# AmmieQi/HGNN-2

Hardware: AMD Instinct MI355X
Metric: graphs/sec forward+backward, QM9-shape batch=512, LG-GNN 5-layer d=64 (higher is better)
Workload: dtype fp32; 1 GPU; GNN_lg order 2, 5 layers, d=64, fwd+bwd, 512 QM9-shape graphs per GPU; graphs_per_gpu=512, global_batch=512, parallelism=dp1

## Files before the change

hgnn-2_amd/csrc/agg.hip:

```cpp
#include "kernels.h"

#include <initializer_list>

namespace hgnn {

template <int CPL, bool V>
__device__ __forceinline__ void load_row(const float* __restrict__ p, int C, int lane, float (&x)[CPL]) {
    const int c0 = lane * CPL;
    if constexpr (V) {
        if constexpr (CPL == 1) {
            x[0] = p[c0];
        } else if constexpr (CPL == 2) {
            const float2 v = *reinterpret_cast<const float2*>(p + c0);
            x[0] = v.x;
            x[1] = v.y;
        } else {
#pragma unroll
            for (int i = 0; i < CPL; i += 4) {
                const float4 v = *reinterpret_cast<const float4*>(p + c0 + i);
                x[i] = v.x;
                x[i + 1] = v.y;
                x[i + 2] = v.z;
                x[i + 3] = v.w;
            }
// ... 206 lines not shown
    if (a.pad_from >= 0) {
        const int kk = a.pad_from > 0 ? a.pad_from : (JT - J0) * a.cg + (CP > 0 ? 2 * a.cp : 0);
        if (lane < a.ldo - kk) o[kk + lane] = 0.f;
    }
}

template <int JT, int CG, int CP, bool V, int RPW, int J0>
__global__ void __launch_bounds__(AGG_NT) k_agg_fwd_rpw(AggFwdArgs a) {
    WaveStamp stamp(a.stamps);
    const int r0 = __builtin_amdgcn_readfirstlane((blockIdx.x * AGG_WV + (threadIdx.x >> 6)) * RPW);
    const int lane = threadIdx.x & 63;
    const int total = *a.total_rows;
    if (r0 >= total) return;
    constexpr int CGx = CG > 0 ? CG : 1, CPx = CP > 0 ? CP : 1, MX = JT > 3 ? JT - 3 : 1;
    RowInfo rgk[RPW], rpk[RPW];
#pragma unroll
    for (int k = 0; k < RPW; ++k) {
        const int r = min(r0 + k, total - 1);
        rgk[k] = RowInfo{0, 0};
        rpk[k] = RowInfo{0, 0};
        if constexpr (CG > 0) rgk[k] = row_info(a.g.rows, r);
        if constexpr (CP > 0) rpk[k] = row_info(a.p.rows, r);
    }
    LaneBn<CGx> bng;
    LaneBn<CPx> bnp;
    if constexpr (CG > 0) bng.init(a.gbn, a.cg, lane);
    if constexpr (CP > 0) bnp.init(a.pbn, a.cp, lane);
    const int stride = a.g.stride;
    float4 mgk[RPW], mpk[RPW];
    float mxk[RPW][MX];
#pragma unroll
    for (int k = 0; k < RPW; ++k) {
        mgk[k] = mpk[k] = make_float4(0.f, 0.f, 0.f, 0.f);
        const int ng = min(64, rgk[k].count), np = min(64, rpk[k].count);
        if constexpr (CG > 0) {
            mgk[k] = lane_entry(a.g.entries, stride, rgk[k].start, ng, lane);
            if constexpr (JT > 3) {
#pragma unroll
                for (int j = 3; j < JT; ++j)
                    mxk[k][j - 3] = lane < ng ? a.g.entries[(long long)(rgk[k].start + lane) * stride + 1 + j] : 0.f;
            }
        }
        if constexpr (CP > 0) mpk[k] = lane_entry(a.p.entries, 4, rpk[k].start, np, lane);
    }
#pragma unroll
    for (int k = 0; k < RPW; ++k) {
    const int r = r0 + k;
    if (r >= total) break;
    const RowInfo rg = rgk[k], rp = rpk[k];
    float* o = a.out + (long long)r * a.ldo;
    float acc[JT][CGx], am[CPx], ad[CPx];
#pragma unroll
    for (int j = 0; j < JT; ++j)
#pragma unroll
        for (int i = 0; i < CGx; ++i) acc[j][i] = 0.f;
#pragma unroll
    for (int i = 0; i < CPx; ++i) am[i] = ad[i] = 0.f;
    const int nmax = max(rg.count, rp.count);
    bool dfound = false;
    for (int e0 = 0; e0 < nmax; e0 += 64) {
        const int ng = min(64, max(0, rg.count - e0)), np = min(64, max(0, rp.count - e0));
        float4 mg = mgk[k], mp = mpk[k];
        float mx[MX];
#pragma unroll
        for (int j = 0; j < MX; ++j) mx[j] = mxk[k][j];
        if (e0 > 0) {
            if constexpr (CG > 0) {
                mg = lane_entry(a.g.entries, stride, rg.start + e0, ng, lane);
                if constexpr (JT > 3) {
#pragma unroll
                    for (int j = 3; j < JT; ++j)
                        mx[j - 3] = lane < ng ? a.g.entries[(long long)(rg.start + e0 + lane) * stride + 1 + j] : 0.f;
                }
            }
            if constexpr (CP > 0) mp = lane_entry(a.p.entries, 4, rp.start + e0, np, lane);
        }
        if constexpr (J0 > 0 && CG > 0)
            if (a.diag) diag_scan(a, r, mg, ng, lane, dfound);
        const int nn = max(ng, np);
        for (int e = 0; e < nn; e += AGG_U) {
            float xg[AGG_U][CGx], v[AGG_U][JT], xp[AGG_U][CPx], vm[AGG_U], vd[AGG_U];
            if constexpr (CG > 0) {
#pragma unroll
                for (int u = 0; u < AGG_U; ++u) {
                    const int eu = max(0, min(e + u, ng - 1));
                    const int col = __builtin_amdgcn_readlane(__float_as_int(mg.x), eu);
                    const bool live = e + u < ng;
                    v[u][0] = live ? bcast(mg.y, eu) : 0.f;
                    if constexpr (JT > 1) v[u][1] = live ? bcast(mg.z, eu) : 0.f;
                    if constexpr (JT > 2) v[u][2] = live ? bcast(mg.w, eu) : 0.f;
#pragma unroll
                    for (int j = 3; j < JT; ++j) v[u][j] = live ? bcast(mx[j - 3], eu) : 0.f;
                    if (ng > 0) load_row<CG, V>(a.xg + (long long)col * a.cg, a.cg, lane, xg[u]);
                    else
#pragma unroll
                        for (int i = 0; i < CG; ++i) xg[u][i] = 0.f;
                }
            }
            if constexpr (CP > 0) {
#pragma unroll
                for (int u = 0; u < AGG_U; ++u) {
                    const int eu = max(0, min(e + u, np - 1));
                    const int col = __builtin_amdgcn_readlane(__float_as_int(mp.x), eu);
                    const bool live = e + u < np;
                    vm[u] = live ? bcast(mp.y, eu) : 0.f;
                    vd[u] = live ? bcast(mp.z, eu) : 0.f;
                    if (np > 0) load_row<CP, V>(a.xp + (long long)col * a.cp, a.cp, lane, xp[u]);
                    else
#pragma unroll
                        for (int i = 0; i < CP; ++i) xp[u][i] = 0.f;
                }
            }
            if constexpr (CG > 0) {
#pragma unroll
                for (int u = 0; u < AGG_U; ++u) bng.apply(xg[u]);
#pragma unroll
                for (int u = 0; u < AGG_U; ++u)
#pragma unroll
                    for (int j = J0; j < JT; ++j)
#pragma unroll
                        for (int i = 0; i < CG; ++i) acc[j][i] = fmaf(v[u][j], xg[u][i], acc[j][i]);
            }
            if constexpr (CP > 0) {
#pragma unroll
                for (int u = 0; u < AGG_U; ++u) bnp.apply(xp[u]);
#pragma unroll
                for (int u = 0; u < AGG_U; ++u)
#pragma unroll
                    for (int i = 0; i < CP; ++i) {
                        am[i] = fmaf(vm[u], xp[u][i], am[i]);
                        ad[i] = fmaf(vd[u], xp[u][i], ad[i]);
                    }
            }
        }
    }
    if constexpr (CG > 0) {
#pragma unroll
        for (int j = J0; j < JT; ++j) store_row<CG, V>(o + (j - J0) * a.cg, a.cg, lane, acc[j]);
        if constexpr (J0 > 0)
            if (a.diag && !dfound && lane == 0) a.diag[r] = make_float2(0.f, 0.f);
    }
    if constexpr (CP > 0) {
        const int base = (JT - J0) * a.cg;
        store_row<CP, V>(o + base, a.cp, lane, am);
        store_row<CP, V>(o + base + a.cp, a.cp, lane, ad);
    }
    if (a.pad_from >= 0) {
        const int kk = a.pad_from > 0 ? a.pad_from : (JT - J0) * a.cg + (CP > 0 ? 2 * a.cp : 0);
        if (lane < a.ldo - kk) o[kk + lane] = 0.f;
    }
    }
}

static int cpl_of(int c) {
    if (c <= 0) return 0;
    if (c <= 64) return 1;
    if (c <= 128) return 2;
    if (c <= 256) return 4;
    if (c <= 512) return 8;
    return -1;
}

template <int JT, int CG, int CP, int J0>
static void agg_fwd_v(const AggFwdArgs& a0, dim3 g, hipStream_t s) {
    AggFwdArgs a = a0;
    const int kk = (JT - J0) * a.cg + (CP > 0 ? 2 * a.cp : 0);
    const bool v = (CG == 0 || vec_ok(CG, a.cg, a.xg, {})) && (CP == 0 || vec_ok(CP, a.cp, a.xp, {})) &&
                   (CG == 0 || vec_ok(CG, a.cg, a.out, {a.ldo, (long long)kk})) &&
                   (CP == 0 || vec_ok(CP, a.cp, a.out, {a.ldo, (long long)(JT - J0) * a.cg, (long long)a.cp}));
    const int rpw = switches().agg_rpw == 3 ? 2 : switches().agg_rpw;
    if constexpr (JT == 3) {
        if (rpw > 1) {
            const dim3 g2(ceil_div(a.cap_rows, rpw * AGG_WV));
            a.stamps = clock_stamps((long long)g2.x * AGG_WV);
            if (rpw == 4) {
                if (v) HGNN_KLAUNCH((k_agg_fwd_rpw<JT, CG, CP, true, 4, J0>), g2, dim3(AGG_NT), 0, s, a);
                else HGNN_KLAUNCH((k_agg_fwd_rpw<JT, CG, CP, false, 4, J0>), g2, dim3(AGG_NT), 0, s, a);
            } else {
                if (v) HGNN_KLAUNCH((k_agg_fwd_rpw<JT, CG, CP, true, 2, J0>), g2, dim3(AGG_NT), 0, s, a);
                else HGNN_KLAUNCH((k_agg_fwd_rpw<JT, CG, CP, false, 2, J0>), g2, dim3(AGG_NT), 0, s, a);
            }
            return;
        }
    }
    a.stamps = clock_stamps((long long)g.x * AGG_WV);
    if (v) HGNN_KLAUNCH((k_agg_fwd<JT, CG, CP, true, J0>), g, dim3(AGG_NT), 0, s, a);
    else HGNN_KLAUNCH((k_agg_fwd<JT, CG, CP, false, J0>), g, dim3(AGG_NT), 0, s, a);
}

template <int JT, int CG, int CP>
static int agg_fwd_j0(const AggFwdArgs& a, dim3 g, hipStream_t s) {
    if (a.j0 == 2) {
        if constexpr (CG > 0 && CG <= 4 && (CP == 0 || CP == CG)) {
            agg_fwd_v<JT, CG, CP, 2>(a, g, s);
            return 0;
        }
        return 2;
    }
    agg_fwd_v<JT, CG, CP, 0>(a, g, s);
    return 0;
}

template <int JT, int CG>
static int agg_fwd_cp(const AggFwdArgs& a, dim3 g, hipStream_t s) {
    int r = 0;
    switch (cpl_of(a.xp ? a.cp : 0)) {
        case 0: r = agg_fwd_j0<JT, CG, 0>(a, g, s); break;
        case 1: r = agg_fwd_j0<JT, CG, 1>(a, g, s); break;
        case 2: r = agg_fwd_j0<JT, CG, 2>(a, g, s); break;
        case 4: r = agg_fwd_j0<JT, CG, 4>(a, g, s); break;
        case 8: r = agg_fwd_j0<JT, CG, 8>(a, g, s); break;
        default: return 2;
    }
    if (r) return r;
    HGNN_LAUNCH_CHECK();
    return 0;
}

template <int JT>
static int agg_fwd_cg(const AggFwdArgs& a, dim3 g, hipStream_t s) {
    switch (cpl_of(a.xg ? a.cg : 0)) {
        case 0:
            if (!a.xp) return 2;
            return agg_fwd_cp<JT, 0>(a, g, s);
        case 1: return agg_fwd_cp<JT, 1>(a, g, s);
        case 2: return agg_fwd_cp<JT, 2>(a, g, s);
        case 4: return agg_fwd_cp<JT, 4>(a, g, s);
        case 8: return agg_fwd_cp<JT, 8>(a, g, s);
        default: return 2;
    }
}

int launch_agg_fwd(const AggFwdArgs& a, hipStream_t s) {
    if (a.cap_rows <= 0) return 0;
    if (a.j0 != 0 && (a.j0 != 2 || !a.xg || (a.diag && !a.err))) return HGNN_ERR_ARG;
    const dim3 g(ceil_div(a.cap_rows, AGG_WV));
    switch (a.jtot) {
        case 3: return agg_fwd_cg<3>(a, g, s);
        case 4: return agg_fwd_cg<4>(a, g, s);
        case 5: return agg_fwd_cg<5>(a, g, s);
        case 6: return agg_fwd_cg<6>(a, g, s);
        case 7: return agg_fwd_cg<7>(a, g, s);
        default: return 2;
    }
}

template <int JT, int C, bool V, int UB>
__device__ __forceinline__ void agg_bwd_g_chunk(const AggBwdArgs& a, float4 me, const float (&mx)[JT > 3 ? JT - 3 : 1],
                                                int n, int lane, float (&acc)[C]) {
    for (int e = 0; e < n; e += UB) {
        float x[UB][JT][C], v[UB][JT];
#pragma unroll
        for (int u = 0; u < UB; ++u) {
            const int eu = min(e + u, n - 1);
            const int col = __builtin_amdgcn_readlane(__float_as_int(me.x), eu);
            const bool live = e + u < n;
            v[u][0] = live ? bcast(me.y, eu) : 0.f;
            if constexpr (JT > 1) v[u][1] = live ? bcast(me.z, eu) : 0.f;
            if constexpr (JT > 2) v[u][2] = live ? bcast(me.w, eu) : 0.f;
#pragma unroll
            for (int j = 3; j < JT; ++j) v[u][j] = live ? bcast(mx[j - 3], eu) : 0.f;
            const float* src = a.ing + (long long)col * a.ldg + a.gofs;
#pragma unroll
            for (int j = 0; j < JT; ++j) {
                if (v[u][j] != 0.f) {
                    load_row<C, V>(src + j * a.c, a.c, lane, x[u][j]);
                } else {
#pragma unroll
                    for (int i = 0; i < C; ++i) x[u][j][i] = 0.f;
                }
            }
        }
#pragma unroll
        for (int u = 0; u < UB; ++u)
#pragma unroll
            for (int j = 0; j < JT; ++j)
#pragma unroll
                for (int i = 0; i < C; ++i) acc[i] = fmaf(v[u][j], x[u][j][i], acc[i]);
    }
}

constexpr int AGG_LONG = 8;

template <int JT, int C, bool V>
__device__ __forceinline__ void agg_bwd_g(const AggBwdArgs& a, int r, int lane) {
    float acc[C];
    float* o = a.out + (long long)r * a.ldo;
    if (a.accumulate) {
        load_row<C, V>(o, a.c, lane, acc);
    } else {
#pragma unroll
        for (int i = 0; i < C; ++i) acc[i] = 0.f;
    }
    const RowInfo ri = row_info(a.g.rows, r);
    const int stride = a.g.stride;
    for (int e0 = 0; e0 < ri.count; e0 += 64) {
        const int n = min(64, ri.count - e0);
        const float4 me = lane_entry(a.g.entries, stride, ri.start + e0, n, lane);
        float mx[JT > 3 ? JT - 3 : 1];
        mx[0] = 0.f;
        if constexpr (JT > 3) {
#pragma unroll
            for (int j = 3; j < JT; ++j)
                mx[j - 3] = lane < n ? a.g.entries[(long long)(ri.start + e0 + lane) * stride + 1 + j] : 0.f;
        }
        if (n > AGG_LONG) agg_bwd_g_chunk<JT, C, V, AGG_LONG>(a, me, mx, n, lane, acc);
        else agg_bwd_g_chunk<JT, C, V, 4>(a, me, mx, n, lane, acc);
    }
    store_row<C, V>(o, a.c, lane, acc);
}

template <int C, bool V>
__device__ __forceinline__ void agg_bwd_p(const AggBwdArgs& a, int r, int lane) {
    float acc[C];
    float* o = a.out + (long long)r * a.ldo;
    if (a.accumulate) {
        load_row<C, V>(o, a.c, lane, acc);
    } else {
#pragma unroll
        for (int i = 0; i < C; ++i) acc[i] = 0.f;
    }
    const RowInfo ri = row_info(a.p.rows, r);
    for (int e0 = 0; e0 < ri.count; e0 += 64) {
        const int n = min(64, ri.count - e0);
        const float4 me = lane_entry(a.p.entries, 4, ri.start + e0, n, lane);
        for (int e = 0; e < n; e += AGG_U) {
            float xm[AGG_U][C], xd[AGG_U][C], vm[AGG_U], vd[AGG_U];
#pragma unroll
            for (int u = 0; u < AGG_U; ++u) {
                const int eu = min(e + u, n - 1);
                const int col = __builtin_amdgcn_readlane(__float_as_int(me.x), eu);
                const bool live = e + u < n;
                vm[u] = live ? bcast(me.y, eu) : 0.f;
                vd[u] = live ? bcast(me.z, eu) : 0.f;
                const float* src = a.inp + (long long)col * a.ldp;
                load_row<C, V>(src + a.pofs_m, a.c, lane, xm[u]);
                load_row<C, V>(src + a.pofs_d, a.c, lane, xd[u]);
            }
#pragma unroll
            for (int u = 0; u < AGG_U; ++u)
#pragma unroll
                for (int i = 0; i < C; ++i) acc[i] = fmaf(vd[u], xd[u][i], fmaf(vm[u], xm[u][i], acc[i]));
        }
    }
    store_row<C, V>(o, a.c, lane, acc);
}

template <int JT, int CG, int CP, bool V, int MODE>
__global__ void __launch_bounds__(AGG_NT) k_agg_bwd(AggBwdArgs ga, AggBwdArgs pa, int gb) {
    WaveStamp stamp(ga.stamps);
    const int lane = threadIdx.x & 63;
    const int wv = threadIdx.x >> 6;
    if (MODE == 1 || (MODE == 3 && (int)blockIdx.x < gb)) {
        if constexpr (MODE != 2) {
            const int r = __builtin_amdgcn_readfirstlane((int)blockIdx.x * AGG_WV + wv);
            if (r >= *ga.total_rows) return;
            agg_bwd_g<JT, CG, V>(ga, r, lane);
        }
    } else {
        if constexpr (MODE != 1) {
            const int r = __builtin_amdgcn_readfirstlane(((int)blockIdx.x - (MODE == 3 ? gb : 0)) * AGG_WV + wv);
            if (r >= *pa.total_rows) return;
            agg_bwd_p<CP, V>(pa, r, lane);
        }
    }
}

static bool bwd_vec_g(int cpl, const AggBwdArgs& a) {
    return vec_ok(cpl, a.c, a.ing, {a.ldg, a.gofs}) && vec_ok(cpl, a.c, a.out, {a.ldo});
}
static bool bwd_vec_p(int cpl, const AggBwdArgs& a) {
    return vec_ok(cpl, a.c, a.inp, {a.ldp, a.pofs_m, a.pofs_d}) && vec_ok(cpl, a.c, a.out, {a.ldo});
}

template <int JT, int C>
static int agg_bwd_single(const AggBwdArgs& a0, hipStream_t s) {
    const dim3 g(ceil_div(a0.cap_rows, AGG_WV));
    AggBwdArgs a = a0;
    a.stamps = clock_stamps((long long)g.x * AGG_WV);
    if (a.ing) {
        if (bwd_vec_g(C, a)) HGNN_KLAUNCH((k_agg_bwd<JT, C, C, true, 1>), g, dim3(AGG_NT), 0, s, a, a, 0);
        else HGNN_KLAUNCH((k_agg_bwd<JT, C, C, false, 1>), g, dim3(AGG_NT), 0, s, a, a, 0);
    } else {
        if (bwd_vec_p(C, a)) HGNN_KLAUNCH((k_agg_bwd<3, C, C, true, 2>), g, dim3(AGG_NT), 0, s, a, a, 0);
        else HGNN_KLAUNCH((k_agg_bwd<3, C, C, false, 2>), g, dim3(AGG_NT), 0, s, a, a, 0);
    }
    HGNN_LAUNCH_CHECK();
    return 0;
}

template <int JT>
static int agg_bwd_c(const AggBwdArgs& a, hipStream_t s) {
    switch (cpl_of(a.c)) {
        case 1: return agg_bwd_single<JT, 1>(a, s);
        case 2: return agg_bwd_single<JT, 2>(a, s);
        case 4: return agg_bwd_single<JT, 4>(a, s);
        case 8: return agg_bwd_single<JT, 8>(a, s);
        default: return 2;
    }
}

int launch_agg_bwd(const AggBwdArgs& a, hipStream_t s) {
    if (a.cap_rows <= 0) return 0;
    if ((a.ing != nullptr) == (a.inp != nullptr)) return 1;
    switch (a.jtot) {
        case 3: return agg_bwd_c<3>(a, s);
        case 4: return agg_bwd_c<4>(a, s);
        case 5: return agg_bwd_c<5>(a, s);
        case 6: return agg_bwd_c<6>(a, s);
        case 7: return agg_bwd_c<7>(a, s);
        default: return 2;
    }
}

template <int JT, int C>
static int agg_bwd_pair_c(const AggBwdArgs& ga0, const AggBwdArgs& pa, hipStream_t s) {
    const int gb = ceil_div(ga0.cap_rows, AGG_WV), pb = ceil_div(pa.cap_rows, AGG_WV);
    AggBwdArgs ga = ga0;
    ga.stamps = clock_stamps((long long)(gb + pb) * AGG_WV);
    HGNN_KLAUNCH((k_agg_bwd<JT, C, C, true, 3>), dim3(gb + pb), dim3(AGG_NT), 0, s, ga, pa, gb);
    HGNN_LAUNCH_CHECK();
    return 0;
}

template <int JT>
static int agg_bwd_pair_j(const AggBwdArgs& ga, const AggBwdArgs& pa, hipStream_t s) {
    switch (cpl_of(ga.c)) {
        case 1: return agg_bwd_pair_c<JT, 1>(ga, pa, s);
        case 2: return agg_bwd_pair_c<JT, 2>(ga, pa, s);
        case 4: return agg_bwd_pair_c<JT, 4>(ga, pa, s);
        case 8: return agg_bwd_pair_c<JT, 8>(ga, pa, s);
        default: return 2;
    }
}

int launch_agg_bwd_pair(const AggBwdArgs& ga, const AggBwdArgs& pa, hipStream_t s) {
    const int cpl = cpl_of(ga.c);
    const bool pair = ga.ing && !ga.inp && pa.inp && !pa.ing && ga.cap_rows > 0 && pa.cap_rows > 0 &&
                      cpl > 0 && cpl == cpl_of(pa.c) && ga.jtot == pa.jtot && bwd_vec_g(cpl, ga) &&
                      bwd_vec_p(cpl, pa);
    if (!pair) {
        int r = launch_agg_bwd(ga, s);
        if (r) return r;
        return launch_agg_bwd(pa, s);
    }
    switch (ga.jtot) {
        case 3: return agg_bwd_pair_j<3>(ga, pa, s);
        case 4: return agg_bwd_pair_j<4>(ga, pa, s);
        case 5: return agg_bwd_pair_j<5>(ga, pa, s);
        case 6: return agg_bwd_pair_j<6>(ga, pa, s);
        case 7: return agg_bwd_pair_j<7>(ga, pa, s);
        default: return 2;
    }
}

}
```

hgnn-2_amd/csrc/bn.hip:

```cpp
#include <algorithm>

#include "kernels.h"

namespace hgnn {

__device__ __forceinline__ double block_sum_d(double v, double* red) {
    v = wave_sum_d(v);
    const int w = threadIdx.x >> 6;
    __syncthreads();
    if ((threadIdx.x & 63) == 0) red[w] = v;
    __syncthreads();
    double t = 0.0;
    const int nw = blockDim.x >> 6;
    for (int i = 0; i < nw; ++i) t += red[i];
    return t;
}

__global__ void __launch_bounds__(256) k_bn_finalize(BnFwdArgs a) {
    WaveStamp stamp(a.stamps);
    const int lane = threadIdx.x & 63;
    const int ch = blockIdx.x * 4 + (threadIdx.x >> 6);
    if (ch >= a.c) return;
    if (!a.training) {
        if (lane == 0) {
// ... 40 lines not shown
            pq[u] = in ? p[2] : 0.f;
        }
    };
    double n = 0.0, sm = 0.0;
    for (int t0 = 0; t0 < tiles; t0 += 64 * U) {
        load(t0);
#pragma unroll
        for (int u = 0; u < U; ++u) {
            n += (double)pn[u];
            sm = fma((double)pn[u], (double)pm[u], sm);
        }
    }
    const double N = wave_total_d(n);
    const double mean = N > 0.0 ? wave_total_d(sm) / N : 0.0;
    double q = 0.0;
    for (int t0 = 0; t0 < tiles; t0 += 64 * U) {
        if (tiles > 64 * U) load(t0);
#pragma unroll
        for (int u = 0; u < U; ++u) {
            const double d = (double)pm[u] - mean;
            q += (double)pq[u] + (double)pn[u] * d * d;
        }
    }
    const double M2 = wave_total_d(q);
    if (lane == 0) {
        const double var = 1e-5 + (N > 0.0 ? M2 / N : 0.0);
        const float mf = (float)mean;
        const float sf = (float)sqrt(var);
        a.mean[ch] = mf;
        a.std[ch] = sf;
        if (a.run_mean) {
            const float m1 = 1.0f - a.momentum;
            a.run_mean[ch] = __fadd_rn(__fmul_rn(m1, mf), __fmul_rn(a.momentum, a.run_mean[ch]));
            a.run_std[ch] = __fadd_rn(__fmul_rn(m1, sf), __fmul_rn(a.momentum, a.run_std[ch]));
        }
    }
}

int launch_bn_finalize(const BnFwdArgs& a, hipStream_t s) {
    BnFwdArgs b = a;
    b.stamps = clock_stamps((long long)ceil_div(a.c, 4) * 4);
    HGNN_KLAUNCH(k_bn_finalize, dim3(ceil_div(a.c, 4)), dim3(256), 0, s, b);
    HGNN_LAUNCH_CHECK();
    return 0;
}

__global__ void __launch_bounds__(256) k_bn_apply(const float* __restrict__ y, const int* total_rows,
                                                  int c, const float* __restrict__ mean,
                                                  const float* __restrict__ stdv, const float* w,
                                                  const float* b, float* __restrict__ z) {
    const long long n = (long long)(*total_rows) * c;
    const float wv = *w, bv = *b;
    for (long long i = (long long)blockIdx.x * blockDim.x + threadIdx.x; i < n;
         i += (long long)gridDim.x * blockDim.x) {
        const int ch = (int)(i % c);
        const float h = __fdiv_rn(__fsub_rn(y[i], mean[ch]), stdv[ch]);
        z[i] = __fadd_rn(__fmul_rn(wv, h), bv);
    }
}

int launch_bn_apply(const float* y, const int* total_rows, int cap_rows, int c, const float* mean,
                    const float* std, const float* w, const float* b, float* z, hipStream_t s) {
    const long long n = (long long)cap_rows * c;
    int blocks = (int)ceil_div<long long>(n, 256);
    if (blocks > 4096) blocks = 4096;
    if (blocks < 1) blocks = 1;
    HGNN_KLAUNCH(k_bn_apply, dim3(blocks), dim3(256), 0, s, y, total_rows, c, mean, std, w, b, z);
    HGNN_LAUNCH_CHECK();
    return 0;
}


__global__ void __launch_bounds__(256) k_bn_bwd_part(BnBwdArgs a) {
    const int tile = blockIdx.x;
    const int total = *a.total_rows;
    const int r0 = tile * 64;
    if (r0 >= total) return;
    const int r1 = min(total, r0 + 64);
    const float wv = *a.w;
    __shared__ float red[4][256];
    const int cw = a.c < 256 ? a.c : 256;
    const int rgn = 256 / cw;
    const int tch = threadIdx.x % cw, rg = threadIdx.x / cw;
    for (int ch0 = 0; ch0 < a.c; ch0 += cw) {
        const int ch = ch0 + tch;
        float s1 = 0.f, s2 = 0.f, t1 = 0.f, t2 = 0.f;
        if (rg < rgn && ch < a.c) {
            const float mu = a.mean[ch], sd = a.std[ch];
            int r = r0 + rg;
            for (; r + 3 * rgn < r1; r += 4 * rgn) {
                float dz[4], yv[4];
#pragma unroll
                for (int u = 0; u < 4; ++u) {
                    const long long i = (long long)(r + u * rgn) * a.c + ch;
                    dz[u] = a.dz[i];
                    yv[u] = a.y[i];
                }
#pragma unroll
                for (int u = 0; u < 4; ++u) {
                    const float h = __fdiv_rn(__fsub_rn(yv[u], mu), sd);
                    const float g = wv * dz[u];
                    s1 += g;
                    s2 = fmaf(g, h, s2);
                    t1 = fmaf(dz[u], h, t1);
                    t2 += dz[u];
                }
            }
            for (; r < r1; r += rgn) {
                const long long i = (long long)r * a.c + ch;
                const float dz = a.dz[i];
                const float h = __fdiv_rn(__fsub_rn(a.y[i], mu), sd);
                const float g = wv * dz;
                s1 += g;
                s2 = fmaf(g, h, s2);
                t1 = fmaf(dz, h, t1);
                t2 += dz;
            }
        }
        red[0][threadIdx.x] = s1;
        red[1][threadIdx.x] = s2;
        red[2][threadIdx.x] = t1;
        red[3][threadIdx.x] = t2;
        __syncthreads();
        if (rg == 0 && ch < a.c) {
            float* p = a.part + bn_bwd_part_index(ch, tile, bn_bwd_tiles(a.cap_rows));
#pragma unroll
            for (int j = 0; j < 4; ++j) {
                float t = 0.f;
                for (int q = 0; q < rgn; ++q) t += red[j][q * cw + tch];
                p[j] = t;
            }
        }
        __syncthreads();
    }
}

__device__ __forceinline__ float4 ld4(const float* p) { return *reinterpret_cast<const float4*>(p); }
__device__ __forceinline__ float& f4c(float4& v, int i) { return reinterpret_cast<float*>(&v)[i]; }

__global__ void __launch_bounds__(256) k_bn_bwd_part4(BnBwdArgs a) {
    WaveStamp stamp(a.stamps);
    const int tile = blockIdx.x;
    const int total = *a.total_rows;
    const int r0 = tile * 64;
    if (r0 >= total) return;
    const int r1 = min(total, r0 + 64);
    const float wv = *a.w;
    const int L = a.c >> 2, RG = min(256 / L, 64);
    const int lane = threadIdx.x % L, rg = threadIdx.x / L;
    __shared__ float4 red[4][256];
    float4 s[4];
#pragma unroll
    for (int j = 0; j < 4; ++j) s[j] = make_float4(0.f, 0.f, 0.f, 0.f);
    if (rg < RG) {
        float mu[4], isd[4];
#pragma unroll
        for (int i = 0; i < 4; ++i) {
            mu[i] = a.mean[4 * lane + i];
            isd[i] = 1.0f / a.std[4 * lane + i];
        }
        auto acc = [&](float4 dz, float4 yv) {
#pragma unroll
            for (int i = 0; i < 4; ++i) {
                const float h = (f4c(yv, i) - mu[i]) * isd[i];
                const float d = f4c(dz, i);
                const float g = wv * d;
                f4c(s[0], i) += g;
                f4c(s[1], i) = fmaf(g, h, f4c(s[1], i));
                f4c(s[2], i) = fmaf(d, h, f4c(s[2], i));
                f4c(s[3], i) += d;
            }
        };
        int r = r0 + rg;
        for (; r + 3 * RG < r1; r += 4 * RG) {
            float4 dz[4], yv[4];
#pragma unroll
            for (int u = 0; u < 4; ++u) {
                const long long i = (long long)(r + u * RG) * a.c + 4 * lane;
                dz[u] = ld4(a.dz + i);
                yv[u] = ld4(a.y + i);
            }
#pragma unroll
            for (int u = 0; u < 4; ++u) acc(dz[u], yv[u]);
        }
        for (; r < r1; r += RG) {
            const long long i = (long long)r * a.c + 4 * lane;
            acc(ld4(a.dz + i), ld4(a.y + i));
        }
    }
#pragma unroll
    for (int j = 0; j < 4; ++j) red[j][threadIdx.x] = s[j];
    __syncthreads();
    for (int ch = threadIdx.x; ch < a.c; ch += 256) {
        const int l = ch >> 2, comp = ch & 3;
        float4 t4;
#pragma unroll
        for (int j = 0; j < 4; ++j) {
            float t = 0.f;
            for (int q = 0; q < RG; ++q) t += f4c(red[j][q * L + l], comp);
            f4c(t4, j) = t;
        }
        if (a.acc64) {
            double* dst = a.acc64 + (long long)(tile % BN_ACC_COPIES) * BN_ACC_STATS * a.c + ch;
#pragma unroll
            for (int j = 0; j < 4; ++j) atomicAdd(dst + (long long)j * a.c, (double)f4c(t4, j));
        } else {
            *reinterpret_cast<float4*>(a.part + bn_bwd_part_index(ch, tile, bn_bwd_tiles(a.cap_rows))) = t4;
        }
    }
}

__device__ __forceinline__ float bn_acc_stat(const double* acc, int c, int j, int ch) {
    double v = 0.0;
#pragma unroll
    for (int q = 0; q < BN_ACC_COPIES; ++q) v += acc[((long long)q * BN_ACC_STATS + j) * c + ch];
    return (float)v;
}

__global__ void __launch_bounds__(256) k_bn_bwd_apply4(BnBwdArgs a) {
    WaveStamp stamp(a.stamps);
    const int total = *a.total_rows;
    const float wv = *a.w;
    const float inv_n = total > 0 ? 1.0f / (float)total : 0.f;
    __shared__ float sm12[2][1024];
    if (a.acc64) {
        for (int ch = threadIdx.x; ch < a.c; ch += blockDim.x) {
            sm12[0][ch] = bn_acc_stat(a.acc64, a.c, 0, ch);
            sm12[1][ch] = bn_acc_stat(a.acc64, a.c, 1, ch);
        }
        if (a.acc64_zero)
            for (long long i = (long long)blockIdx.x * blockDim.x + threadIdx.x; i < bn_acc_doubles(a.c);
                 i += (long long)gridDim.x * blockDim.x)
                a.acc64_zero[i] = 0.0;
        __syncthreads();
    }
    if (blockIdx.x == 0) {
        __shared__ double redd[4];
        double t1 = 0.0, t2 = 0.0;
        for (int ch = threadIdx.x; ch < a.c; ch += blockDim.x) {
            t1 += (double)(a.acc64 ? bn_acc_stat(a.acc64, a.c, 2, ch) : a.sums[ch * 4 + 2]);
            t2 += (double)(a.acc64 ? bn_acc_stat(a.acc64, a.c, 3, ch) : a.sums[ch * 4 + 3]);
        }
        const double T1 = block_sum_d(t1, redd);
        const double T2 = block_sum_d(t2, redd);
        if (threadIdx.x == 0) {
            *a.dw = (float)T1;
            *a.db = (float)T2;
        }
    }
    const int r0 = blockIdx.x * 64;
    if (r0 >= total) return;
    const int r1 = min(total, r0 + 64);
    const int L = a.c >> 2, RG = min(256 / L, 64);
    const int lane = threadIdx.x % L, rg = threadIdx.x / L;
    __shared__ float4 red[256];
    float4 cs = make_float4(0.f, 0.f, 0.f, 0.f);
    if (rg < RG) {
        float mu[4], isd[4], m1[4], m2[4];
        bool relu[4];
#pragma unroll
        for (int i = 0; i < 4; ++i) {
            const int ch = 4 * lane + i;
            mu[i] = a.mean[ch];
            isd[i] = 1.0f / a.std[ch];
            m1[i] = (a.acc64 ? sm12[0][ch] : a.sums[ch * 4 + 0]) * inv_n;
            m2[i] = (a.acc64 ? sm12[1][ch] : a.sums[ch * 4 + 1]) * inv_n;
            relu[i] = ch >= a.relu_from;
        }
        auto one = [&](long long i, float4 yv, float4 dz) {
            float4 d;
#pragma unroll
            for (int k = 0; k < 4; ++k) {
                f4c(d, k) = bn_bwd_dy_inv(f4c(yv, k), f4c(dz, k), mu[k], isd[k], wv, m1[k], m2[k], a.training != 0,
                                          relu[k]);
                f4c(cs, k) += f4c(d, k);
            }
            *reinterpret_cast<float4*>(a.dy + i) = d;
        };
        int r = r0 + rg;
        for (; r + 7 * RG < r1; r += 8 * RG) {
            float4 dz[8], yv[8];
#pragma unroll
            for (int u = 0; u < 8; ++u) {
                const long long i = (long long)(r + u * RG) * a.c + 4 * lane;
                dz[u] = ld4(a.dz + i);
                yv[u] = ld4(a.y + i);
            }
#pragma unroll
            for (int u = 0; u < 8; ++u) one((long long)(r + u * RG) * a.c + 4 * lane, yv[u], dz[u]);
        }
        for (; r + 3 * RG < r1; r += 4 * RG) {
            float4 dz[4], yv[4];
#pragma unroll
            for (int u = 0; u < 4; ++u) {
                const long long i = (long long)(r + u * RG) * a.c + 4 * lane;
                dz[u] = ld4(a.dz + i);
                yv[u] = ld4(a.y + i);
            }
#pragma unroll
            for (int u = 0; u < 4; ++u) one((long long)(r + u * RG) * a.c + 4 * lane, yv[u], dz[u]);
        }
        for (; r < r1; r += RG) {
            const long long i = (long long)r * a.c + 4 * lane;
            one(i, ld4(a.y + i), ld4(a.dz + i));
        }
    }
    if (a.dbpart) {
        red[threadIdx.x] = cs;
        __syncthreads();
        for (int ch = threadIdx.x; ch < a.c; ch += 256) {
            const int l = ch >> 2, comp = ch & 3;
            float t = 0.f;
            for (int q = 0; q < RG; ++q) t += f4c(red[q * L + l], comp);
            a.dbpart[(long long)blockIdx.x * a.c + ch] = t;
        }
    }
}

static bool bn_vec4(const BnBwdArgs& a) {
    const uintptr_t al = reinterpret_cast<uintptr_t>(a.y) | reinterpret_cast<uintptr_t>(a.dz) |
                         reinterpret_cast<uintptr_t>(a.dy);
    return a.c > 0 && a.c % 4 == 0 && a.c <= 1024 && (al & 15) == 0;
}

__global__ void __launch_bounds__(256) k_bn_bwd_fin(BnBwdArgs a) {
    WaveStamp stamp(a.stamps);
    const int lane = threadIdx.x & 63;
    const int ch = blockIdx.x * 4 + (threadIdx.x >> 6);
    if (ch >= a.c) return;
    const int tiles = ceil_div(*a.total_rows, 64);
    const int ntl = bn_bwd_tiles(a.cap_rows);
    constexpr int U = 8;
    double v[4] = {0.0, 0.0, 0.0, 0.0};
    for (int t0 = 0; t0 < tiles; t0 += 64 * U) {
        float4 pv[U];
#pragma unroll
        for (int u = 0; u < U; ++u) {
            const int t = min(t0 + u * 64 + lane, max(tiles - 1, 0));
            pv[u] = *reinterpret_cast<const float4*>(a.part + bn_bwd_part_index(ch, t, ntl));
        }
#pragma unroll
        for (int u = 0; u < U; ++u)
            if (t0 + u * 64 + lane < tiles) {
                v[0] += (double)pv[u].x;
                v[1] += (double)pv[u].y;
                v[2] += (double)pv[u].z;
                v[3] += (double)pv[u].w;
            }
    }
#pragma unroll
    for (int j = 0; j < 4; ++j) v[j] = wave_total_d(v[j]);
    if (lane == 0) {
#pragma unroll
        for (int j = 0; j < 4; ++j) a.sums[ch * 4 + j] = (float)v[j];
    }
}

__global__ void __launch_bounds__(256) k_bn_bwd_apply(BnBwdArgs a) {
    const int total = *a.total_rows;
    const long long n = (long long)total * a.c;
    const float wv = *a.w;
    const float inv_n = total > 0 ? 1.0f / (float)total : 0.f;
    if (blockIdx.x == 0) {
        __shared__ double red[4];
        double t1 = 0.0, t2 = 0.0;
        for (int ch = threadIdx.x; ch < a.c; ch += blockDim.x) {
            t1 += (double)a.sums[ch * 4 + 2];
            t2 += (double)a.sums[ch * 4 + 3];
        }
        const double T1 = block_sum_d(t1, red);
        const double T2 = block_sum_d(t2, red);
        if (threadIdx.x == 0) {
            *a.dw = (float)T1;
            *a.db = (float)T2;
        }
    }
    (void)n;
    __shared__ float red[256];
    const int r0 = blockIdx.x * 64;
    if (r0 >= total) return;
    const int r1 = min(total, r0 + 64);
    const int ldy = a.ldy > 0 ? a.ldy : a.c;
    for (int e = threadIdx.x; e < (r1 - r0) * (ldy - a.c); e += blockDim.x)
        a.dy[(long long)(r0 + e / (ldy - a.c)) * ldy + a.c + e % (ldy - a.c)] = 0.f;
    const int cw = a.c < 256 ? a.c : 256;
    const int rgn = 256 / cw;
    const int tch = threadIdx.x % cw, rg = threadIdx.x / cw;
    for (int ch0 = 0; ch0 < a.c; ch0 += cw) {
        const int ch = ch0 + tch;
        float cs = 0.f;
        if (rg < rgn && ch < a.c) {
            const float sd = a.std[ch];
            const float mu = a.mean[ch];
            const float m1 = a.sums[ch * 4 + 0] * inv_n;
            const float m2 = a.sums[ch * 4 + 1] * inv_n;
            auto one = [&](float yv, float dzv) {
                return bn_bwd_dy(yv, dzv, mu, sd, wv, m1, m2, a.training != 0, ch >= a.relu_from);
            };
            int r = r0 + rg;
            for (; r + 3 * rgn < r1; r += 4 * rgn) {
                float yv[4], dzv[4];
#pragma unroll
                for (int u = 0; u < 4; ++u) {
                    const long long i = (long long)(r + u * rgn) * a.c + ch;
                    yv[u] = a.y[i];
                    dzv[u] = a.dz[i];
                }
#pragma unroll
                for (int u = 0; u < 4; ++u) {
                    const float d = one(yv[u], dzv[u]);
                    a.dy[(long long)(r + u * rgn) * ldy + ch] = d;
                    cs += d;
                }
            }
            for (; r < r1; r += rgn) {
                const long long i = (long long)r * a.c + ch;
                const float d = one(a.y[i], a.dz[i]);
                a.dy[(long long)r * ldy + ch] = d;
                cs += d;
            }
        }
        if (a.dbpart) {
            red[threadIdx.x] = cs;
            __syncthreads();
            if (rg == 0 && ch < a.c) {
                float t = 0.f;
                for (int q = 0; q < rgn; ++q) t += red[q * cw + tch];
                a.dbpart[(long long)blockIdx.x * a.c + ch] = t;
            }
            __syncthreads();
        }
    }
}

constexpr int BN2_THREADS = 1024, BN2_ROWS = 256;

template <int L>
__device__ __forceinline__ float4 wave_groups_sum4(float4 v) {
#pragma unroll
    for (int o = L; o < 64; o <<= 1) {
        v.x += __shfl_xor(v.x, o, 64);
        v.y += __shfl_xor(v.y, o, 64);
        v.z += __shfl_xor(v.z, o, 64);
        v.w += __shfl_xor(v.w, o, 64);
    }
    return v;
}

__device__ __forceinline__ float4 f4_zero() { return make_float4(0.f, 0.f, 0.f, 0.f); }

template <int L, int LS = L>
__global__ void __launch_bounds__(BN2_THREADS) k_bn_bwd_part2(BnBwdArgs a) {
    constexpr int RG = BN2_THREADS / L, RPT = BN2_ROWS / RG, C = 4 * LS;
    const int tile = blockIdx.x;
    const int total = *a.total_rows;
    const int r0 = tile * BN2_ROWS;
    if (r0 >= total) return;
    const int r1 = min(total, r0 + BN2_ROWS);
    const float wv = *a.w;
    const int c0 = blockIdx.y * 4 * L;
    const int lane = threadIdx.x % L, rg = threadIdx.x / L;
    float mu[4], isd[4];
#pragma unroll
    for (int i = 0; i < 4; ++i) {
        mu[i] = a.mean[c0 + 4 * lane + i];
        isd[i] = 1.0f / a.std[c0 + 4 * lane + i];
    }
// ... 731 lines not shown
```

Before: 506,700 graphs/s.

## Add narrow-channel aggregation kernels packing 8 rows per wave; prefetch BN bwd tiles

Adds forward and backward sparse aggregation kernels for channel counts of at most 8. Each wave handles 8 rows with 8 lanes per row, loads entry metadata cooperatively and broadcasts it via shuffles, where before one wave covered a single row and most lanes sat idle. The BN backward kernels now issue their first tile of dz/y loads before the shared-memory stats setup, and move the block-0 reduction to the end so those loads overlap with the prologue. This adds several kernel variants and more complex masking logic. It also changes the order of the backward reduction, which can shift floating-point results slightly.

Result: faster. 515,400 graphs/s (median of 6 runs) (+1.7%).

```diff
diff --git a/hgnn-2_amd/csrc/agg.hip b/hgnn-2_amd/csrc/agg.hip
--- a/hgnn-2_amd/csrc/agg.hip
+++ b/hgnn-2_amd/csrc/agg.hip
@@ -382,6 +382,159 @@
     }
 }
 
+#ifndef AGG_NARROW
+#define AGG_NARROW 1
+#endif
+constexpr int AGG_NLPR = 8, AGG_NGPW = 64 / AGG_NLPR, AGG_NU = 4;
+
+__device__ __forceinline__ RowInfo row_info_lane(const RowInfo* rows, int r) {
+    const int2 v = *reinterpret_cast<const int2*>(reinterpret_cast<const int*>(rows) + 2 * (long long)r);
+    return RowInfo{v.x, v.y};
+}
+
+struct NarrowList {
+    int base, cnt, wmax;
+    __device__ __forceinline__ void init(RowInfo ri) {
+        cnt = ri.count;
+        const unsigned long long m = __ballot(ri.count > 0);
+        const int fs = __shfl(ri.start, m ? __ffsll(m) - 1 : 0, 64);
+        base = ri.count > 0 ? ri.start : fs;
+        int w = max(ri.count, 0);
+#pragma unroll
+        for (int o = AGG_NLPR; o < 64; o <<= 1) w = max(w, __shfl_xor(w, o, 64));
+        wmax = __builtin_amdgcn_readfirstlane(w);
+    }
+    __device__ __forceinline__ long long at(int e0, int i, bool& live) const {
+        live = e0 + i < cnt;
+        return (long long)base + min(e0 + i, max(cnt - 1, 0));
+    }
+};
+
+__device__ __forceinline__ float grp_bcast(float v, int src) { return __shfl(v, src, 64); }
+__device__ __forceinline__ float f4_at(const float4& v, int i) { return i == 0 ? v.x : i == 1 ? v.y : i == 2 ? v.z : v.w; }
+
+template <int JT, bool HG, bool HP>
+__global__ void __launch_bounds__(AGG_NT) k_agg_fwd_narrow(AggFwdArgs a) {
+    WaveStamp stamp(a.stamps);
+    const int r0 = __builtin_amdgcn_readfirstlane((blockIdx.x * AGG_WV + (threadIdx.x >> 6)) * AGG_NGPW);
+    const int lane = threadIdx.x & 63, i = lane & (AGG_NLPR - 1), g0 = lane & ~(AGG_NLPR - 1);
+    const int total = *a.total_rows;
+    if (r0 >= total) return;
+    const int r = r0 + (lane >> 3);
+    const int rc = min(r, total - 1);
+    NarrowList gl{0, 0, 0}, pl{0, 0, 0};
+    {
+        RowInfo rg{0, 0}, rp{0, 0};
+        if constexpr (HG) rg = row_info_lane(a.g.rows, rc);
+        if constexpr (HP) rp = row_info_lane(a.p.rows, rc);
+        if constexpr (HG) gl.init(rg);
+        if constexpr (HP) pl.init(rp);
+    }
+    const int ig = min(i, max(a.cg - 1, 0)), ip = min(i, max(a.cp - 1, 0));
+    const bool gbn = HG && a.gbn.mean != nullptr, pbn = HP && a.pbn.mean != nullptr;
+    float gmu = 0.f, gsc = 1.f, gb = 0.f, pmu = 0.f, psc = 1.f, pb = 0.f;
+    if (gbn) gmu = a.gbn.mean[ig], gsc = bn_scale(*a.gbn.w, a.gbn.std[ig]), gb = *a.gbn.b;
+    if (pbn) pmu = a.pbn.mean[ip], psc = bn_scale(*a.pbn.w, a.pbn.std[ip]), pb = *a.pbn.b;
+    const int stride = a.g.stride;
+    float acc[JT], am = 0.f, ad = 0.f;
+#pragma unroll
+    for (int j = 0; j < JT; ++j) acc[j] = 0.f;
+    const int nmax = max(gl.wmax, pl.wmax);
+    for (int e0 = 0; e0 < nmax; e0 += AGG_NLPR) {
+        const bool gon = HG && e0 < gl.wmax, pon = HP && e0 < pl.wmax;
+        float4 mg = make_float4(0.f, 0.f, 0.f, 0.f), mp = mg, mx4 = mg;
+        if (gon) {
+            bool live;
+            const float* q = a.g.entries + gl.at(e0, i, live) * stride;
+            mg = *reinterpret_cast<const float4*>(q);
+            if constexpr (JT > 3) mx4 = *reinterpret_cast<const float4*>(q + 4);
+            if (!live) {
+                mg.y = mg.z = mg.w = 0.f;
+                mx4 = make_float4(0.f, 0.f, 0.f, 0.f);
+            }
+        }
+        if (pon) {
+            bool live;
+            mp = *reinterpret_cast<const float4*>(a.p.entries + pl.at(e0, i, live) * 4);
+            if (!live) mp.y = mp.z = 0.f;
+        }
+        const int nn = min(AGG_NLPR, nmax - e0);
+        for (int e = 0; e < nn; e += AGG_NU) {
+            float xg[AGG_NU], v[AGG_NU][JT], xp[AGG_NU], vm[AGG_NU], vd[AGG_NU];
+#pragma unroll
+            for (int u = 0; u < AGG_NU; ++u) {
+                const int src = g0 + e + u;
+                xg[u] = xp[u] = 0.f;
+#pragma unroll
+                for (int j = 0; j < JT; ++j) v[u][j] = 0.f;
+                vm[u] = vd[u] = 0.f;
+                if (gon) {
+                    const int col = __float_as_int(grp_bcast(mg.x, src));
+                    v[u][0] = grp_bcast(mg.y, src);
+                    if constexpr (JT > 1) v[u][1] = grp_bcast(mg.z, src);
+                    if constexpr (JT > 2) v[u][2] = grp_bcast(mg.w, src);
+#pragma unroll
+                    for (int j = 3; j < JT; ++j) v[u][j] = grp_bcast(f4_at(mx4, j - 3), src);
+                    xg[u] = a.xg[(long long)col * a.cg + ig];
+                }
+                if (pon) {
+                    const int col = __float_as_int(grp_bcast(mp.x, src));
+                    vm[u] = grp_bcast(mp.y, src);
+                    vd[u] = grp_bcast(mp.z, src);
+                    xp[u] = a.xp[(long long)col * a.cp + ip];
+                }
+            }
+            if (gon) {
+#pragma unroll
+                for (int u = 0; u < AGG_NU; ++u) {
+                    if (gbn) xg[u] = bn_z_s(xg[u], gmu, gsc, gb);
+#pragma unroll
+                    for (int j = 0; j < JT; ++j) acc[j] = fmaf(v[u][j], xg[u], acc[j]);
+                }
+            }
+            if (pon) {
+#pragma unroll
+                for (int u = 0; u < AGG_NU; ++u) {
+                    if (pbn) xp[u] = bn_z_s(xp[u], pmu, psc, pb);
+                    am = fmaf(vm[u], xp[u], am);
+                    ad = fmaf(vd[u], xp[u], ad);
+                }
+            }
+        }
+    }
+    if (r >= total) return;
+    float* o = a.out + (long long)r * a.ldo;
+    if constexpr (HG) {
+        if (i < a.cg) {
+#pragma unroll
+            for (int j = 0; j < JT; ++j) o[j * a.cg + i] = acc[j];
+        }
+    }
+    if constexpr (HP) {
+        const int base = JT * a.cg;
+        if (i < a.cp) {
+            o[base + i] = am;
+            o[base + a.cp + i] = ad;
+        }
+    }
+    if (a.pad_from >= 0) {
+        const int kk = a.pad_from > 0 ? a.pad_from : JT * a.cg + (HP ? 2 * a.cp : 0);
+        for (int p = kk + i; p < a.ldo; p += AGG_NLPR) o[p] = 0.f;
+    }
+}
+
+template <int JT>
+static int agg_fwd_narrow(const AggFwdArgs& a0, bool hg, bool hp, hipStream_t s) {
+    AggFwdArgs a = a0;
+    const dim3 g(ceil_div(ceil_div(a.cap_rows, AGG_NGPW), AGG_WV));
+    a.stamps = clock_stamps((long long)g.x * AGG_WV);
+    if (hg && hp) HGNN_KLAUNCH((k_agg_fwd_narrow<JT, true, true>), g, dim3(AGG_NT), 0, s, a);
+    else if (hg) HGNN_KLAUNCH((k_agg_fwd_narrow<JT, true, false>), g, dim3(AGG_NT), 0, s, a);
+    else HGNN_KLAUNCH((k_agg_fwd_narrow<JT, false, true>), g, dim3(AGG_NT), 0, s, a);
+    HGNN_LAUNCH_CHECK();
+    return 0;
+}
+
 static int cpl_of(int c) {
     if (c <= 0) return 0;
     if (c <= 64) return 1;
@@ -465,6 +618,17 @@
     if (a.cap_rows <= 0) return 0;
     if (a.j0 != 0 && (a.j0 != 2 || !a.xg || (a.diag && !a.err))) return HGNN_ERR_ARG;
     const dim3 g(ceil_div(a.cap_rows, AGG_WV));
+    const int cgn = a.xg && a.cg > 0 ? a.cg : 0, cpn = a.xp && a.cp > 0 ? a.cp : 0;
+    if (AGG_NARROW && a.j0 == 0 && cgn <= AGG_NLPR && cpn <= AGG_NLPR && (cgn > 0 || cpn > 0)) {
+        switch (a.jtot) {
+            case 3: return agg_fwd_narrow<3>(a, cgn > 0, cpn > 0, s);
+            case 4: return agg_fwd_narrow<4>(a, cgn > 0, cpn > 0, s);
+            case 5: return agg_fwd_narrow<5>(a, cgn > 0, cpn > 0, s);
+            case 6: return agg_fwd_narrow<6>(a, cgn > 0, cpn > 0, s);
+            case 7: return agg_fwd_narrow<7>(a, cgn > 0, cpn > 0, s);
+            default: return 2;
+        }
+    }
     switch (a.jtot) {
         case 3: return agg_fwd_cg<3>(a, g, s);
         case 4: return agg_fwd_cg<4>(a, g, s);
@@ -594,6 +758,83 @@
             agg_bwd_p<CP, V>(pa, r, lane);
         }
     }
+}
+
+template <int JT, int MODE>
+__global__ void __launch_bounds__(AGG_NT) k_agg_bwd_narrow(AggBwdArgs a) {
+    WaveStamp stamp(a.stamps);
+    const int r0 = __builtin_amdgcn_readfirstlane((blockIdx.x * AGG_WV + (threadIdx.x >> 6)) * AGG_NGPW);
+    const int lane = threadIdx.x & 63, i = lane & (AGG_NLPR - 1), g0 = lane & ~(AGG_NLPR - 1);
+    const int total = *a.total_rows;
+    if (r0 >= total) return;
+    const int r = r0 + (lane >> 3);
+    const int rc = min(r, total - 1);
+    const int ic = min(i, a.c - 1);
+    float acc = 0.f;
+    if (a.accumulate) acc = a.out[(long long)rc * a.ldo + ic];
+    NarrowList l;
+    l.init(row_info_lane(MODE == 1 ? a.g.rows : a.p.rows, rc));
+    const int cnt = max(l.cnt, 0), rem = cnt & 63;
+    const int ub = MODE == 1 && rem > AGG_LONG ? AGG_LONG : 4;
+    const int proc = (cnt - rem) + (rem + ub - 1) / ub * ub;
+    const int stride = MODE == 1 ? a.g.stride : 4;
+    const float* entries = MODE == 1 ? a.g.entries : a.p.entries;
+    for (int e0 = 0; e0 < l.wmax; e0 += AGG_NLPR) {
+        bool live;
+        const float* q = entries + l.at(e0, i, live) * stride;
+        float4 me = *reinterpret_cast<const float4*>(q), mx4 = make_float4(0.f, 0.f, 0.f, 0.f);
+        if constexpr (MODE == 1 && JT > 3) mx4 = *reinterpret_cast<const float4*>(q + 4);
+        if (!live) {
+            me.y = me.z = me.w = 0.f;
+            mx4 = make_float4(0.f, 0.f, 0.f, 0.f);
+        }
+        const int nn = min(AGG_NLPR, l.wmax - e0);
+        for (int e = 0; e < nn; e += AGG_NU) {
+            constexpr int NS = MODE == 1 ? JT : 2;
+            float x[AGG_NU][NS], v[AGG_NU][NS];
+#pragma unroll
+            for (int u = 0; u < AGG_NU; ++u) {
+                const int src = g0 + e + u;
+                const int col = __float_as_int(grp_bcast(me.x, src));
+                v[u][0] = grp_bcast(me.y, src);
+                v[u][1] = grp_bcast(me.z, src);
+                if constexpr (MODE == 1) {
+                    if constexpr (JT > 2) v[u][2] = grp_bcast(me.w, src);
+#pragma unroll
+                    for (int j = 3; j < JT; ++j) v[u][j] = grp_bcast(f4_at(mx4, j - 3), src);
+                    const float* s = a.ing + (long long)col * a.ldg + a.gofs + ic;
+#pragma unroll
+                    for (int j = 0; j < JT; ++j) x[u][j] = s[j * a.c];
+                } else {
+                    const float* s = a.inp + (long long)col * a.ldp + ic;
+                    x[u][0] = s[a.pofs_m];
+                    x[u][1] = s[a.pofs_d];
+                }
+            }
+#pragma unroll
+            for (int u = 0; u < AGG_NU; ++u) {
+                float t = acc;
+#pragma unroll
+                for (int j = 0; j < NS; ++j) {
+                    const float xv = MODE == 1 && v[u][j] == 0.f ? 0.f : x[u][j];
+                    t = fmaf(v[u][j], xv, t);
+                }
+                acc = e0 + e + u < proc ? t : acc;
+            }
+        }
+    }
+    if (r < total && i < a.c) a.out[(long long)r * a.ldo + i] = acc;
+}
+
+template <int JT>
+static int agg_bwd_narrow(const AggBwdArgs& a0, hipStream_t s) {
+    const dim3 g(ceil_div(ceil_div(a0.cap_rows, AGG_NGPW), AGG_WV));
+    AggBwdArgs a = a0;
+    a.stamps = clock_stamps((long long)g.x * AGG_WV);
+    if (a.ing) HGNN_KLAUNCH((k_agg_bwd_narrow<JT, 1>), g, dim3(AGG_NT), 0, s, a);
+    else HGNN_KLAUNCH((k_agg_bwd_narrow<3, 2>), g, dim3(AGG_NT), 0, s, a);
+    HGNN_LAUNCH_CHECK();
+    return 0;
 }
 
 static bool bwd_vec_g(int cpl, const AggBwdArgs& a) {
@@ -621,6 +862,7 @@
 
 template <int JT>
 static int agg_bwd_c(const AggBwdArgs& a, hipStream_t s) {
+    if (AGG_NARROW && a.c > 0 && a.c <= AGG_NLPR) return agg_bwd_narrow<JT>(a, s);
     switch (cpl_of(a.c)) {
         case 1: return agg_bwd_single<JT, 1>(a, s);
         case 2: return agg_bwd_single<JT, 2>(a, s);
diff --git a/hgnn-2_amd/csrc/bn.hip b/hgnn-2_amd/csrc/bn.hip
--- a/hgnn-2_amd/csrc/bn.hip
+++ b/hgnn-2_amd/csrc/bn.hip
@@ -216,6 +216,15 @@
     float4 s[4];
 #pragma unroll
     for (int j = 0; j < 4; ++j) s[j] = make_float4(0.f, 0.f, 0.f, 0.f);
+    constexpr int U0 = 8;
+    float4 dz0[U0], yv0[U0];
+#pragma unroll
+    for (int u = 0; u < U0; ++u) {
+        if (u * RG >= 64) break;
+        const long long i = (long long)min(r0 + rg + u * RG, r1 - 1) * a.c + 4 * lane;
+        dz0[u] = ld4(a.dz + i);
+        yv0[u] = ld4(a.y + i);
+    }
     if (rg < RG) {
         float mu[4], isd[4];
 #pragma unroll
@@ -236,6 +245,10 @@
             }
         };
         int r = r0 + rg;
+#pragma unroll
+        for (int u = 0; u < U0; ++u)
+            if (r + u * RG < r1) acc(dz0[u], yv0[u]);
+        r += U0 * RG;
         for (; r + 3 * RG < r1; r += 4 * RG) {
             float4 dz[4], yv[4];
 #pragma unroll
@@ -286,6 +299,28 @@
     const int total = *a.total_rows;
     const float wv = *a.w;
     const float inv_n = total > 0 ? 1.0f / (float)total : 0.f;
+    const int r0 = blockIdx.x * 64;
+    const bool tile = r0 < total;
+    const int r1 = min(total, r0 + 64);
+    const int L = a.c >> 2, RG = min(256 / L, 64);
+    const int lane = threadIdx.x % L, rg = threadIdx.x / L;
+    constexpr int U0 = 8;
+    float4 dz0[U0], yv0[U0];
+    float mu[4], sd[4];
+    if (tile) {
+#pragma unroll
+        for (int u = 0; u < U0; ++u) {
+            if (u * RG >= 64) break;
+            const long long i = (long long)min(r0 + rg + u * RG, r1 - 1) * a.c + 4 * lane;
+            dz0[u] = ld4(a.dz + i);
+            yv0[u] = ld4(a.y + i);
+        }
+#pragma unroll
+        for (int i = 0; i < 4; ++i) {
+            mu[i] = a.mean[4 * lane + i];
+            sd[i] = a.std[4 * lane + i];
+        }
+    }
     __shared__ float sm12[2][1024];
     if (a.acc64) {
         for (int ch = threadIdx.x; ch < a.c; ch += blockDim.x) {
@@ -298,35 +333,15 @@
                 a.acc64_zero[i] = 0.0;
         __syncthreads();
     }
-    if (blockIdx.x == 0) {
-        __shared__ double redd[4];
-        double t1 = 0.0, t2 = 0.0;
-        for (int ch = threadIdx.x; ch < a.c; ch += blockDim.x) {
-            t1 += (double)(a.acc64 ? bn_acc_stat(a.acc64, a.c, 2, ch) : a.sums[ch * 4 + 2]);
-            t2 += (double)(a.acc64 ? bn_acc_stat(a.acc64, a.c, 3, ch) : a.sums[ch * 4 + 3]);
-        }
-        const double T1 = block_sum_d(t1, redd);
-        const double T2 = block_sum_d(t2, redd);
-        if (threadIdx.x == 0) {
-            *a.dw = (float)T1;
-            *a.db = (float)T2;
-        }
-    }
-    const int r0 = blockIdx.x * 64;
-    if (r0 >= total) return;
-    const int r1 = min(total, r0 + 64);
-    const int L = a.c >> 2, RG = min(256 / L, 64);
-    const int lane = threadIdx.x % L, rg = threadIdx.x / L;
     __shared__ float4 red[256];
     float4 cs = make_float4(0.f, 0.f, 0.f, 0.f);
-    if (rg < RG) {
-        float mu[4], isd[4], m1[4], m2[4];
+    if (tile && rg < RG) {
+        float isd[4], m1[4], m2[4];
         bool relu[4];
 #pragma unroll
         for (int i = 0; i < 4; ++i) {
             const int ch = 4 * lane + i;
-            mu[i] = a.mean[ch];
-            isd[i] = 1.0f / a.std[ch];
+            isd[i] = 1.0f / sd[i];
             m1[i] = (a.acc64 ? sm12[0][ch] : a.sums[ch * 4 + 0]) * inv_n;
             m2[i] = (a.acc64 ? sm12[1][ch] : a.sums[ch * 4 + 1]) * inv_n;
             relu[i] = ch >= a.relu_from;
@@ -342,6 +357,10 @@
             *reinterpret_cast<float4*>(a.dy + i) = d;
         };
         int r = r0 + rg;
+#pragma unroll
+        for (int u = 0; u < U0; ++u)
+            if (r + u * RG < r1) one((long long)(r + u * RG) * a.c + 4 * lane, yv0[u], dz0[u]);
+        r += U0 * RG;
         for (; r + 7 * RG < r1; r += 8 * RG) {
             float4 dz[8], yv[8];
 #pragma unroll
@@ -369,7 +388,7 @@
             one(i, ld4(a.y + i), ld4(a.dz + i));
         }
     }
-    if (a.dbpart) {
+    if (tile && a.dbpart) {
         red[threadIdx.x] = cs;
         __syncthreads();
         for (int ch = threadIdx.x; ch < a.c; ch += 256) {
@@ -377,6 +396,20 @@
             float t = 0.f;
             for (int q = 0; q < RG; ++q) t += f4c(red[q * L + l], comp);
             a.dbpart[(long long)blockIdx.x * a.c + ch] = t;
+        }
+    }
+    if (blockIdx.x == 0) {
+        __shared__ double redd[4];
+        double t1 = 0.0, t2 = 0.0;
+        for (int ch = threadIdx.x; ch < a.c; ch += blockDim.x) {
+            t1 += (double)(a.acc64 ? bn_acc_stat(a.acc64, a.c, 2, ch) : a.sums[ch * 4 + 2]);
+            t2 += (double)(a.acc64 ? bn_acc_stat(a.acc64, a.c, 3, ch) : a.sums[ch * 4 + 3]);
+        }
+        const double T1 = block_sum_d(t1, redd);
+        const double T2 = block_sum_d(t2, redd);
+        if (threadIdx.x == 0) {
+            *a.dw = (float)T1;
+            *a.db = (float)T2;
         }
     }
 }
```
